# pengpeng-yu/FastPCC

Measured on AMD Instinct MI355X. Metric: encode+decode Mpoints/sec, lossy_coord_v2 baseline_r1 (stream of 16-frame batches, 2 in flight; one frame at a time = value_one_frame), higher is better.
Workload: dtype f32; 1 GPU; lossy_coord_v2/baseline_r1 inference, 997645-voxel 1024^3 body-surface frames (cfg#2), seeded random-init weights; one step = a batch of 16 such frames per GPU (15966320 voxels) through compress_many + decompress_many = ONE network traversal over the batch, 16 independent streams; 2 batch(es) in flight per GPU; parallelism=single GPU, 2 batches in flight per GPU on one stream (fastpcc_amd/serving.py), batch_clouds=16, frames_in_flight=2, named_stages=False, bytes=143901, coder_handover_retries=0

## Files before the change

fastpcc_amd/csrc/hip/conv.hip:

```cpp
#include "conv_common.h"
#include <atomic>
#include <cstdlib>

namespace fpcc {
namespace {

template <int NBT, int CH, int WM, int WN>
struct MfmaCfg {
    static constexpr int C_OUT = 32 * NBT;
    static constexpr int TM = 32 * WM;
    static constexpr int NBW = NBT / WN;
    static constexpr int THREADS = 64 * WM * WN;
    static constexpr int G8 = CH / 8;
    static constexpr int W_TOTAL = CH * C_OUT / 4;
    static constexpr int W_PIECES = (W_TOTAL + THREADS - 1) / THREADS;
    static_assert(NBT % WN == 0, "column blocks must divide over the waves");
};

template <typename C, int CH>
__device__ __forceinline__ void fetch_a(const ConvArgs &a, const int32_t *nbr_rows, int cc, int li, int lh,
                                        f32x4 (&ra)[C::G8]) {
    const bool in_x1 = cc * CH < a.c1;
    const float *xb = in_x1 ? a.x1 + cc * CH : a.x2 + (cc * CH - a.c1);
    const int64_t ld = in_x1 ? a.ld1 : a.ld2;
    const int32_t idx = nbr_rows[li];
// ... 1591 lines not shown
    }
    if (ch == 32) {
        if (c_out == 128) return launch_mfma<4, 32>(a, s);
        if (c_out == 64) return launch_mfma<2, 32>(a, s);
        return launch_mfma<1, 32>(a, s);
    }
    if (ch == 16) {
        if (c_out == 128) return launch_mfma<4, 16>(a, s);
        if (c_out == 64) return launch_mfma<2, 16>(a, s);
        return launch_mfma<1, 16>(a, s);
    }
    if (c1 == 1 && c2 == 0 && n_offsets == 1 && !nbr && groups == 1 && !out_map && c_out >= 8) {
        hipLaunchKernelGGL(k_conv_c1_pointwise, dim3(blocks_for(n_out * c_out, 256)), dim3(256), 0, s, a);
        return check_hip(hipGetLastError(), "k_conv_c1_pointwise");
    }
    if (c_out == 1) return launch_valu<1>(a, s);
    if (c_out <= 4) return launch_valu<4>(a, s);
    if (c_out <= 8) return launch_valu<8>(a, s);
    return launch_valu<16>(a, s);
}

namespace fpcc {
namespace {
__global__ void k_conv_row_keys(const int32_t *__restrict__ nbr, int n_off, int64_t nbr_ks, int64_t nbr_os, int64_t n,
                                int window_log2, int64_t *__restrict__ keys, uint32_t *__restrict__ masks) {
    const int64_t o = (int64_t)blockIdx.x * blockDim.x + threadIdx.x;
    if (o >= n) return;
    uint32_t m = 0;
    for (int k = 0; k < n_off; ++k) m |= (nbr[(int64_t)k * nbr_ks + o * nbr_os] >= 0 ? 1u : 0u) << k;
    if (masks) masks[o] = m;
    m ^= m >> 1; m ^= m >> 2; m ^= m >> 4; m ^= m >> 8; m ^= m >> 16;
    keys[o] = ((o >> window_log2) << 32) | (int64_t)m;
}

__global__ void k_conv_row_keys_masks(const uint32_t *__restrict__ masks, int64_t n, int window_log2, int64_t *__restrict__ keys) {
    const int64_t o = (int64_t)blockIdx.x * blockDim.x + threadIdx.x;
    if (o >= n) return;
    uint32_t m = masks[o];
    m ^= m >> 1; m ^= m >> 2; m ^= m >> 4; m ^= m >> 8; m ^= m >> 16;
    keys[o] = ((o >> window_log2) << 32) | (int64_t)m;
}

__global__ __launch_bounds__(256) void k_gather_table_rows(const int4 *__restrict__ rows, const int32_t *__restrict__ order, int64_t n,
                                                           int pieces, int4 *__restrict__ out) {
    const int64_t e = (int64_t)blockIdx.x * 256 + threadIdx.x;
    if (e >= n * pieces) return;
    const int64_t p = e / pieces;
    const int j = (int)(e - p * pieces);
    out[e] = rows[(int64_t)order[p] * pieces + j];
}

__global__ __launch_bounds__(256) void k_conv_tile_keys(const uint32_t *__restrict__ row_masks, int n_off,
                                                        const int32_t *__restrict__ row_order, int64_t n, int group,
                                                        int64_t n_groups, int64_t *__restrict__ keys) {
    const int64_t g = (int64_t)blockIdx.x * 4 + (threadIdx.x >> 6);
    const int lane = threadIdx.x & 63;
    if (g >= n_groups) return;
    const int64_t pos = g * group + lane;
    uint32_t m = 0;
    if (lane < group && pos < n) m = row_masks[row_order ? (int64_t)row_order[pos] : pos];
#pragma unroll
    for (int o = 32; o > 0; o >>= 1) m |= __shfl_xor(m, o);
    if (lane == 0) keys[g] = ((int64_t)(n_off - __popc(m)) << 32) | g;
}
// ... 41 lines not shown
    __syncthreads();
#pragma unroll
    for (int j = 0; j < kPer; ++j) {
        if (bin[j] == 255) continue;
        uint32_t pos = 0;
#pragma unroll
        for (int b = 0; b < kBins; ++b)
            if (bin[j] == b) { pos = s_base[b] + s_wave[wv][b] + before[b]; before[b] += 1; }
        perm[pos] = g0 + j;
    }
}

__global__ void k_conv_regroup_rows(const int32_t *__restrict__ row_order, const int32_t *__restrict__ group_perm, int64_t n,
                                    int group, int64_t n_groups, int32_t *__restrict__ out) {
    const int64_t p = (int64_t)blockIdx.x * blockDim.x + threadIdx.x;
    if (p >= n) return;
    const int64_t g = p / group;
    const int64_t src = g < n_groups ? (int64_t)group_perm[g] * group + (p - g * group) : p;
    out[p] = row_order ? row_order[src] : (int32_t)src;
}
}
}

extern "C" int fpcc_conv_tile_keys(const uint32_t *row_masks, int n_offsets, const int32_t *row_order, int64_t n, int group,
                                   int64_t *keys_out, void *stream) {
    if (n < 0 || n_offsets < 1 || n_offsets > 32 || group < 1 || group > 64) return fail_arg("conv_tile_keys: sizes out of range");
    const int64_t n_groups = n / group;
    if (n_groups == 0) return FPCC_OK;
    if (!row_masks || !keys_out) return fail_arg("conv_tile_keys: null pointer");
    hipLaunchKernelGGL(k_conv_tile_keys, dim3(blocks_for(n_groups, 4)), dim3(256), 0, as_stream(stream), row_masks, n_offsets,
                       row_order, n, group, n_groups, keys_out);
    return check_hip(hipGetLastError(), "k_conv_tile_keys");
}

extern "C" int fpcc_conv_group_order(const int64_t *group_keys, int64_t n_groups, int32_t *perm_out, void *stream) {
    if (n_groups < 0 || n_groups > 16384) return fail_arg("conv_group_order: at most 16384 groups");
    if (n_groups == 0) return FPCC_OK;
    if (!group_keys || !perm_out) return fail_arg("conv_group_order: null pointer");
    const int per = (int)((n_groups + 1023) / 1024);
    if (per <= 2) hipLaunchKernelGGL(k_group_counting_order<2>, dim3(1), dim3(1024), 0, as_stream(stream), group_keys, (int)n_groups, perm_out);
    else if (per <= 5) hipLaunchKernelGGL(k_group_counting_order<5>, dim3(1), dim3(1024), 0, as_stream(stream), group_keys, (int)n_groups, perm_out);
    else hipLaunchKernelGGL(k_group_counting_order<16>, dim3(1), dim3(1024), 0, as_stream(stream), group_keys, (int)n_groups, perm_out);
    return check_hip(hipGetLastError(), "k_group_counting_order");
}

extern "C" int fpcc_conv_regroup_rows(const int32_t *row_order, const int32_t *group_perm, int64_t n, int group,
                                      int32_t *row_order_out, void *stream) {
    if (n < 0 || group < 1) return fail_arg("conv_regroup_rows: sizes out of range");
    if (n == 0) return FPCC_OK;
    if (!row_order_out || (n / group > 0 && !group_perm)) return fail_arg("conv_regroup_rows: null pointer");
    hipLaunchKernelGGL(k_conv_regroup_rows, dim3(blocks_for(n, 256)), dim3(256), 0, as_stream(stream), row_order, group_perm, n,
                       group, n / group, row_order_out);
    return check_hip(hipGetLastError(), "k_conv_regroup_rows");
}

extern "C" int fpcc_conv_row_keys_masks(const uint32_t *masks, int64_t n, int window_log2, int64_t *keys_out, void *stream) {
    if (n < 0 || window_log2 < 5 || window_log2 > 31) return fail_arg("conv_row_keys_masks: bad sizes");
    if (n == 0) return FPCC_OK;
    if (!masks || !keys_out) return fail_arg("conv_row_keys_masks: null pointer");
    hipLaunchKernelGGL(k_conv_row_keys_masks, dim3(blocks_for(n, 256)), dim3(256), 0, as_stream(stream), masks, n, window_log2, keys_out);
    return check_hip(hipGetLastError(), "k_conv_row_keys_masks");
}

extern "C" int fpcc_gather_table_rows_i32(const int32_t *rows, int ld, const int32_t *order, int64_t n, int32_t *out, void *stream) {
    if (n < 0 || ld < 4 || ld % 4) return fail_arg("gather_table_rows: ld must be a positive multiple of 4");
    if (n == 0) return FPCC_OK;
    if (!rows || !order || !out || !aligned16(rows) || !aligned16(out)) return fail_arg("gather_table_rows: null or unaligned pointer");
    hipLaunchKernelGGL(k_gather_table_rows, dim3(blocks_for(n * (ld / 4), 256)), dim3(256), 0, as_stream(stream),
                       reinterpret_cast<const int4 *>(rows), order, n, ld / 4, reinterpret_cast<int4 *>(out));
    return check_hip(hipGetLastError(), "k_gather_table_rows");
}

extern "C" int fpcc_conv_row_keys(const int32_t *nbr, int n_offsets, int64_t nbr_ks, int64_t nbr_os, int64_t n,
                                  int window_log2, int64_t *keys_out, uint32_t *masks_out, void *stream) {
    if (n < 0 || n_offsets < 1 || n_offsets > 32 || window_log2 < 5 || window_log2 > 30)
        return fail_arg("conv_row_keys: sizes out of range");
    if (n == 0) return FPCC_OK;
    if (!nbr || !keys_out) return fail_arg("conv_row_keys: null pointer");
    hipLaunchKernelGGL(k_conv_row_keys, dim3(blocks_for(n, 256)), dim3(256), 0, as_stream(stream), nbr, n_offsets, nbr_ks,
                       nbr_os, n, window_log2, keys_out, masks_out);
    return check_hip(hipGetLastError(), "k_conv_row_keys");
}

namespace fpcc {
namespace {
constexpr int64_t kK2s2tSparseRows = 200 * 1024;
std::atomic<long long> g_k2s2t_sparse_launches{0};

__global__ __launch_bounds__(1024) void k_k2s2t_order(const int32_t *__restrict__ parent_of, const int32_t *__restrict__ child_row,
                                                      int64_t n, int64_t n_parents, int window_log2, int32_t *__restrict__ order,
                                                      int32_t *__restrict__ table) {
    __shared__ uint32_t s_cnt[16][8];
    __shared__ uint32_t s_base[2][8];
    const int t = threadIdx.x, lane = t & 63, wv = t >> 6;
    const int64_t w0 = (int64_t)blockIdx.x << window_log2;
    const int64_t w1 = min(n, w0 + ((int64_t)1 << window_log2));
    auto octant_of = [&](int64_t c, int32_t &par) {
        par = parent_of[c];
        if (par < 0 || par >= n_parents) { par = -1; return 0; }
        const int4 *line = reinterpret_cast<const int4 *>(child_row + (int64_t)par * 8);
        const int4 lo = line[0], hi = line[1];
        const int32_t e[8] = {lo.x, lo.y, lo.z, lo.w, hi.x, hi.y, hi.z, hi.w};
        int o = -1;
#pragma unroll
// ... 234 lines not shown
```

fastpcc_amd/engine.py:

```python
import functools
import math
import os
from enum import Enum
from typing import Dict, List, Optional, Sequence, Tuple, Union

import torch
import torch.nn as nn

from . import hipops as ops
from .autograd import conv_autocast


class RegionType(Enum):
    HYPER_CUBE = 0
    HYPER_CROSS = 1
    CUSTOM = 2


class MinkowskiAlgorithm(Enum):
    DEFAULT = 0
    MEMORY_EFFICIENT = 1
    SPEED_OPTIMIZED = 2


# ... 152 lines not shown
            raise KeyError(f'{key} is not in this coordinate manager') from None

    def get_coordinate_map_keys(self, tensor_stride) -> List[CoordinateMapKey]:
        s = _as_stride(tensor_stride)
        return [k for k in self._maps if k._stride == s]

    def insert_and_map(self, coordinates: torch.Tensor, tensor_stride=1, string_id: str = ''):
        stride = _as_stride(tensor_stride)
        level = stride[0].bit_length() - 1
        if coordinates.dtype != torch.int32 or coordinates.dim() != 2 or coordinates.shape[1] != 4:
            raise TypeError('coordinates must be int32 [n, 4] = (batch, x, y, z)')
        coordinates = coordinates.contiguous()
        self.device = coordinates.device
        if self._bits0 is None:
            nb = self._n_batch
            if nb is None:
                nb = int(coordinates[:, 0].max().item()) + 1 if coordinates.shape[0] else 1
            self._n_batch = nb
            self._bits0 = min(21, (63 - max(nb - 1, 0).bit_length()) // 3)
        bits = self._bits0 - level
        if bits < 1:
            raise ValueError('tensor stride exceeds the coordinate range')
        keys = ops.keys_from_coords(coordinates, level, bits)
        skeys, perm = ops.sort_keys(keys, 63)
        ukeys, first, count = ops.unique_keys(skeys)
        n = int(count.item())
        m = _Map(level, bits, n, ukeys[:n])
        rows = perm if n == coordinates.shape[0] else perm[first[:n].long()]
        key = self._register(m, string_id)
        return key, (rows, n)

    def _ensure_parent(self, m: _Map, rows: Optional[int] = None, edges: Optional[List[int]] = None) -> _Map:
        if m.parent is None:
            if m.bits <= 1:
                raise ValueError('cannot stride past the coordinate range')
            parent_of, pkeys, child_row, count = ops.coarsen(self._keys(m))
            cnt = int(count.item()) if rows is None else rows
            p = _Map(m.level + 1, m.bits - 1, cnt, pkeys[:cnt])
            p.edges = edges
            m.parent, m.parent_of, m.child_row = p, parent_of, child_row[:cnt]
            self._register(p, '')
        return m.parent

    def build_pyramid(self, key: CoordinateMapKey, levels: int) -> None:
        m = self._map(key)
        while m.parent is not None and levels > 0:
            m, levels = m.parent, levels - 1
# ... 94 lines not shown
        return dict(nbr=m.nbr27_pos, n_offsets=27, nbr_ks=1, nbr_os=32)

    def _mask27(self, m: _Map) -> Optional[torch.Tensor]:
        if m.mask27 is None:
            if m.generated or m.nbr27 is not None:
                return None
            if m.parent is None and m.n > self.ROOT_ROWS and m.bits > 1:
                self._ensure_parent(m)
            if m.parent is None:
                return None
            m.mask27 = ops.mask27_from_parent(m.keys, m.parent_of, self._nbr27(m.parent, True), m.child_row)
        return m.mask27

    ROW_ORDER_MIN_ROWS = int(os.environ.get('FPCC_ROW_ORDER_MIN_ROWS', '8192'))
    ROW_ORDER_WINDOW_LOG2 = int(os.environ.get('FPCC_ROW_WINDOW_LOG2', '19'))

    ROW_ORDER_MIN_ROWS_TRAINING = 512

    def _row_order(self, m: _Map, training: bool = False) -> Optional[torch.Tensor]:
        if m.row_order is False or (m.row_order is None and training and m.n > self.ROW_ORDER_MIN_ROWS_TRAINING):
            m.row_order = None
            if m.n > (self.ROW_ORDER_MIN_ROWS_TRAINING if training else self.ROW_ORDER_MIN_ROWS):
                nbr = self._nbr27(m, want_rows=not training)
                m.row_order = ops.conv_row_order(nbr, 27, m.n, 1, m.n, self.ROW_ORDER_WINDOW_LOG2,
                                                 masks=m.mask27 if m.nbr27_rows is not None else None)
        return m.row_order

    def _k2_order(self, src: _Map):
        m = src.parent.n
        if src.k2_order is False:
            src.k2_order = None
            if self.NBR_ROWS and m > self.ROW_ORDER_MIN_ROWS and os.environ.get('FPCC_K2_ROW_ORDER', '1') != '0':
                src.k2_order = ops.conv_row_order(src.child_row, 8, 1, 8, m, self.ROW_ORDER_WINDOW_LOG2)
                src.k2_pos = ops.gather_table_rows(src.child_row, src.k2_order)
        if src.k2_order is None:
            return None, src.child_row
        return src.k2_order, src.k2_pos

    K2T_WINDOW_LOG2 = ops.K2S2T_WINDOW_LOG2

    def _k2t_order(self, dst: _Map):
        if dst.k2t_order is False:
            dst.k2t_order = None
            po, cr = dst.parent_of, dst.child_row
            if dst.n > 0 and po is not None and cr is not None and dst.parent is not None and po.numel() == dst.n and \
                    po.dtype == torch.int32 and cr.dtype == torch.int32 and cr.dim() == 2 and tuple(cr.shape) == (dst.parent.n, 8) and \
                    po.is_contiguous() and cr.is_contiguous():
                dst.k2t_order, dst.k2t_table = ops.conv_k2s2t_order(po, cr, dst.n, self.K2T_WINDOW_LOG2)
        return dst.k2t_order, dst.k2t_table

    def get_coordinates(self, key: CoordinateMapKey) -> torch.Tensor:
        m = self._map(key)
        if m.coords is None:
            m.coords = ops.coords_from_keys(self._keys(m), m.level, m.bits)
        return m.coords

    def kernel_map(self, in_key: CoordinateMapKey, out_key: CoordinateMapKey, stride=1, kernel_size=1, **_):
# ... 625 lines not shown
```

fastpcc_amd/hipops.py:

```python
import collections
import ctypes as C
import functools
from typing import List, Optional, Sequence, Tuple

import torch

from . import _native

_vp, _i64, _i32, _f32 = C.c_void_p, C.c_int64, C.c_int, C.c_float

ACT_NONE, ACT_PRELU, ACT_RELU = 0, 1, 2

_SIGS = {
    'fpcc_morton3d_encode': (_i32, [_vp, _i64, _i64, _i32, _i32, _i32, _vp, _vp]),
    'fpcc_hilbert3d_encode': (_i32, [_vp, _i64, _i64, _i32, _i32, _i32, _i32, _vp, _vp]),
    'fpcc_keys_from_coords': (_i32, [_vp, _i64, _i32, _i32, _vp, _vp]),
    'fpcc_coords_from_keys': (_i32, [_vp, _i64, _i32, _i32, _vp, _vp, _vp]),
    'fpcc_sort_keys': (_i64, [_vp, _i64, _i32, _vp, _vp, _vp, _i64, _vp]),
    'fpcc_unique_keys': (_i64, [_vp, _i64, _vp, _vp, _vp, _vp, _i64, _vp]),
    'fpcc_coarsen': (_i64, [_vp, _i64, _vp, _vp, _vp, _vp, _vp, _i64, _vp]),
    'fpcc_octree_level': (_i64, [_vp, _i64, _i64, _i32, _vp, _vp, _vp, _vp, _i64, _vp, _vp, _i64, _vp]),
    'fpcc_level_histogram': (_i64, [_vp, _i64, _i32, _vp, _vp]),
    'fpcc_level_histogram_clouds': (_i64, [_vp, _i64, _i32, _i32, _i32, _vp, _vp]),
    'fpcc_refine': (_i64, [_vp, _i64, _vp, _vp, _vp, _vp, _vp, _vp, _i64, _vp]),
    'fpcc_nbr27_search': (_i32, [_vp, _i64, _i32, _vp, _vp]),
    'fpcc_nbr27_from_parent': (_i32, [_vp, _vp, _i64, _vp, _i64, _vp, _vp, _vp]),
    'fpcc_nbr27_from_parent_ex': (_i32, [_vp, _vp, _i64, _vp, _i64, _vp, _vp, _vp, _vp, _vp]),
    'fpcc_conv_row_keys_masks': (_i32, [_vp, _i64, _i32, _vp, _vp]),
    'fpcc_gather_table_rows_i32': (_i32, [_vp, _i32, _vp, _i64, _vp, _vp]),
    'fpcc_mask27_from_parent': (_i32, [_vp, _vp, _i64, _vp, _i64, _vp, _vp, _vp]),
    'fpcc_conv_ones_k3_f32': (_i32, [_vp, _i64, _vp, _vp, _i32, _i32, _vp, C.c_float, _vp, _i32, _vp]),
    'fpcc_conv_f32': (_i32, [_vp, _i32, _i32, _vp, _i32, _i32, _vp, _i32, _i64, _i64, _vp, _vp, _i32, _i32,
                             _vp, _i64, _i64, _vp, _i32, _i64, _i32, _vp, _f32, _vp, _vp, _i64, _vp]),
    'fpcc_conv_f32_pk': (_i32, [_vp, _i32, _i32, _vp, _i32, _i32, _vp, _i32, _i64, _i64, _vp, _vp, _vp, _i32, _i32,
                                _vp, _i64, _i64, _vp, _i32, _i64, _i32, _vp, _f32, _vp, _vp, _i64, _vp]),
    'fpcc_conv_set_tuning': (_i32, [_i32, _i32]),
    'fpcc_conv_fold64_launches': (_i64, []),
    'fpcc_conv_k2s2t_order': (_i32, [_vp, _vp, _i64, _i64, _i32, _vp, _vp, _vp]),
    'fpcc_conv_k2s2t_f32': (_i32, [_vp, _i32, _i32, _vp, _vp, _vp, _vp, _i32, _vp, _i32, _i64, _i32, _vp, _f32, _vp]),
    'fpcc_conv_k2s2t_use_sparse': (_i32, [_i32, _i32, _i64]),
    'fpcc_conv_k2s2t_sparse_launches': (_i64, []),
    'fpcc_conv_debug_stamps': (_i32, [_vp, _i64]),
    'fpcc_conv_i8_debug_stamps': (_i32, [_vp, _i64]),
    'fpcc_time_next_launch': (_i32, [_vp, _vp]),
    'fpcc_transpose_table_i32': (_i32, [_vp, _i32, _i64, _vp, _i32, _vp]),
    'fpcc_numerics_version': (_i32, []),
    'fpcc_conv_packed_floats': (_i64, [_i32, _i32, _i32, _i32, _i32]),
    'fpcc_conv_pack_weights_f32': (_i32, [_vp, _i64, _i32, _i32, _vp, _vp]),
    'fpcc_conv_f32_natural_matrix': (_i32, [_i32, _i32, _i32, _i32, _i32]),
    'fpcc_conv_packed_floats_nat': (_i64, [_i32, _i32, _i32, _i32, _i32]),
    'fpcc_conv_pack_weights_nat_f32': (_i32, [_vp, _i64, _i32, _i32, _vp, _vp]),
# ... 2 lines not shown
    'fpcc_nn_dist2': (_i32, [_vp, _i64, _i32, _vp, _i64, _vp, _vp, _vp]),
    'fpcc_knn3d': (_i32, [_vp, _i64, _vp, _i64, _i32, _vp, _vp, _vp]),
    'fpcc_sum_i64': (_i32, [_vp, _i64, _vp, _vp]),
    'fpcc_knn_voxels': (_i32, [_vp, _i64, _i32, _vp, _i64, _i32, _i32, _vp, _vp, _vp]),
    'fpcc_pca_normals': (_i32, [_vp, _i64, _i32, _vp, _i64, _i32, _vp, _vp]),
    'fpcc_nn_plane_dist2': (_i32, [_vp, _i64, _i32, _vp, _vp, _i64, _vp, _vp, _vp, _vp]),
    'fpcc_transfer_normals_ws_bytes': (_i64, [_i64, _i64]),
    'fpcc_transfer_normals': (_i32, [_vp, _i64, _vp, _vp, _vp, _i64, _vp, _i32, _vp, _vp, _i64, _vp]),
    'fpcc_sum_max_f64': (_i32, [_vp, _i64, _vp, _vp, _i64, _vp]),
    'fpcc_recolor_ws_bytes': (_i64, [_i64]),
    'fpcc_recolor': (_i32, [_vp, _i64, _vp, _i64, _vp, _i32, _vp, _vp, _i64, _vp]),
    'fpcc_keys_member': (_i32, [_vp, _i64, _vp, _i64, _vp, _vp]),
    'fpcc_transpose_weights_f32': (_i32, [_vp, _i32, _i32, _i32, _i32, _vp, _vp]),
    'fpcc_conv_wgrad_ws_bytes': (_i64, [_i32, _i32, _i32, _i32, _i64]),
    'fpcc_conv_wgrad_f32': (_i32, [_vp, _i32, _i32, _vp, _i32, _i32, _vp, _i32, _i64, _i64, _vp, _i64, _i64, _i32, _i64, _vp, _vp,
                                   _i32, _vp, _i64, _vp]),
    'fpcc_conv_wgrad_matrix': (_i32, [_i32, _i32]),
    'fpcc_epilogue_bwd_ws_bytes': (_i64, [_i64, _i32]),
    'fpcc_epilogue_bwd_f32': (_i32, [_vp, _i32, _vp, _i32, _i64, _i32, _i32, _vp, _vp, _i32, _vp, _vp, _vp, _i64, _vp]),
    'fpcc_noisy_normal_ws_bytes': (_i64, [_i64]),
    'fpcc_noisy_normal_bits_f32': (_i32, [_vp, _vp, _i64, _f32, _f32, _f32, _vp, _vp, _vp, _vp, _i64, _vp]),
    'fpcc_deep_factorized_ws_bytes': (_i64, [_i64, _i32]),
    'fpcc_deep_factorized_bits_f32': (_i32, [_vp, _i64, _i32, _i32, _vp, _vp, _vp, _f32, _vp, _i32, _vp, _vp, _i64, _vp]),
    'fpcc_conv_tile_keys': (_i32, [_vp, _i32, _vp, _i64, _i32, _vp, _vp]),
    'fpcc_conv_regroup_rows': (_i32, [_vp, _vp, _i64, _i32, _vp, _vp]),
    'fpcc_conv_group_order': (_i32, [_vp, _i64, _vp, _vp]),
    'fpcc_conv_row_keys': (_i32, [_vp, _i32, _i64, _i64, _i64, _i32, _vp, _vp, _vp]),
    'fpcc_conv_f32_ws_bytes': (_i64, [_i32, _i32, _i32, _i32, _i32, _i64]),
    'fpcc_conv_f32_order': (_i32, [_i32, _i32, _i32]),
    'fpcc_conv_f32_order_ex': (_i32, [_i32, _i32, _i32, _i32, _i32, _i64]),
    'fpcc_conv_f32_plan': (_i32, [_i32, _i32, _i32, _i32, _i32, _vp]),
    'fpcc_gather_sum_f32': (_i32, [_vp, _i32, _vp, _i32, _i64, _i64, _i64, _vp, _i32, _vp, _f32, _vp, _vp]),
    'fpcc_gather_sum_generated_f32': (_i32, [_vp, _i32, _vp, _i64, _vp, _i32, _vp, _f32, _vp, _vp]),
    'fpcc_logit_to_prob16': (_i32, [_vp, _i64, _vp, _vp]),
    'fpcc_quantize_symbols': (_i32, [_vp, _i64, _f32, _vp, _vp]),
    'fpcc_child_mask': (_i32, [_vp, _i64, _vp, _vp]),
    'fpcc_topk_keep': (_i64, [_vp, _i64, _i64, _vp, _vp, _i64, _vp]),
    'fpcc_topk_keep_cells': (_i64, [_vp, _i64, _vp, _i64, _i64, _vp, _vp, _i64, _vp]),
    'fpcc_topk_keep_batch': (_i64, [_vp, _i64, _vp, _i32, _vp, _i64, _vp, _vp, _vp, _i64, _vp]),
    'fpcc_gather_rows_f32': (_i32, [_vp, _i32, _i32, _vp, _i64, _vp, _i32, _vp]),
    'fpcc_compact_coords': (_i64, [_vp, _i64, _vp, _i32, _i32, _vp, _vp, _vp, _vp, _i64, _vp]),
    'fpcc_int_init': (_i32, []),
    'fpcc_hash_insert_coords': (_i32, [_vp, _vp, _i64, _vp, _i64, _vp]),
    'fpcc_hash_lookup_coords': (_i32, [_vp, _vp, _i64, _vp, _i64, _vp, _vp, _vp, _vp]),
    'fpcc_hash_insert_coords_bxyz': (_i32, [_vp, _vp, _i64, _vp, _i64, _vp]),
    'fpcc_hash_lookup_coords_bxyz': (_i32, [_vp, _vp, _i64, _vp, _i64, _vp, _vp, _vp, _vp]),
    'fpcc_hash_insert_keys': (_i32, [_vp, _vp, _i64, _vp, _i64, _vp]),
    'fpcc_hash_lookup_keys': (_i32, [_vp, _vp, _i64, _vp, _i64, _vp, _vp]),
    'fpcc_conv_i8': (_i32, [_vp, _i32, _i32, _vp, _i32, _i64, _i64, _i32, _vp, _i32, _vp, _vp, _vp, _vp, _vp, _i32, _i32,
                            _vp, _i32, _i32, _i32, _i64, _vp, _vp, _i64, _vp]),
# ... 931 lines not shown
                                        None if dy is None else dy.data_ptr(), c, out.data_ptr(), ws.data_ptr(), need, _stream()))
    return out, dy


def noisy_normal_bits(y: torch.Tensor, index: torch.Tensor, log_scale_offset: float, log_scale_factor: float,
                      half_width: float = 0.5):
    n = y.numel()
    if index.numel() != n:
        raise ValueError('one index per value')
    index = index.to(torch.float32)
    py, pi = _dev(y, torch.float32, 'y', n == 0), _dev(index, torch.float32, 'index', n == 0)
    dy = torch.empty(n, dtype=torch.float32, device=y.device)
    di = torch.empty(n, dtype=torch.float32, device=y.device)
    out = torch.empty(1, dtype=torch.float32, device=y.device)
    L = lib()
    need = _ok(L.fpcc_noisy_normal_ws_bytes(n))
    ws = torch.empty(max(need // 4, 1), dtype=torch.float32, device=y.device)
    _ok(L.fpcc_noisy_normal_bits_f32(py, pi, n, float(log_scale_offset), float(log_scale_factor), float(half_width),
                                     dy.data_ptr(), di.data_ptr(), out.data_ptr(), ws.data_ptr(), need, _stream()))
    return out[0], dy, di


def conv_row_order(nbr: Optional[torch.Tensor], n_offsets: int, nbr_ks: int, nbr_os: int, n: int, window_log2: int = 13,
                   heaviest_first: bool = True, masks: Optional[torch.Tensor] = None) -> torch.Tensor:
    L = lib()
    dev = masks.device if masks is not None else nbr.device
    keys = torch.empty(n, dtype=torch.int64, device=dev)
    group = 64 if n >= 32 * 1024 else 32
    n_groups = n // group
    heaviest_first = heaviest_first and 2 <= n_groups <= LPT_MAX_GROUPS
    if masks is not None:
        _ok(L.fpcc_conv_row_keys_masks(_dev(masks, torch.int32, 'masks'), n, window_log2, keys.data_ptr(), _stream()))
    else:
        masks = torch.empty(n, dtype=torch.int32, device=dev) if heaviest_first else None
        _ok(L.fpcc_conv_row_keys(_dev(nbr, torch.int32, 'nbr'), n_offsets, nbr_ks, nbr_os, n, window_log2, keys.data_ptr(),
                                 None if masks is None else masks.data_ptr(), _stream()))
    order = sort_keys(keys, 32 + max(1, (n >> window_log2).bit_length()))[1]
    if not heaviest_first:
        return order
    gkeys = torch.empty(n_groups, dtype=torch.int64, device=dev)
    _ok(L.fpcc_conv_tile_keys(masks.data_ptr(), n_offsets, order.data_ptr(), n, group, gkeys.data_ptr(), _stream()))
    gperm = torch.empty(n_groups, dtype=torch.int32, device=dev)
    _ok(L.fpcc_conv_group_order(gkeys.data_ptr(), n_groups, gperm.data_ptr(), _stream()))
    out = torch.empty_like(order)
    _ok(L.fpcc_conv_regroup_rows(order.data_ptr(), gperm.data_ptr(), n, group, out.data_ptr(), _stream()))
    return out


LPT_MAX_GROUPS = 1 << 14

def table_conv_chunk(c_in: int, c_out: int, k: int) -> int:
    mfma = conv_order(c_in, 0, c_out, 1, 1, 0) != 0
    if not mfma:
        return 32
    return k if k <= 27 else 16


class ConvPlan(C.Structure):
    _fields_ = [('order', _i32), ('matrix', _i32), ('packed', _i32), ('chunk', _i32), ('packed_floats', _i64), ('ws_bytes', _i64)]


ConvPlanValue = collections.namedtuple('ConvPlanValue', [f for f, _ in ConvPlan._fields_])


@functools.lru_cache(maxsize=8192)
def conv_plan(c1: int, c2: int, c_out: int, n_offsets: int = 1, groups: int = 1) -> ConvPlanValue:
    plan = ConvPlan()
    _ok(lib().fpcc_conv_f32_plan(c1, c2, c_out, n_offsets, groups, C.byref(plan)))
    return ConvPlanValue(*(getattr(plan, f) for f in ConvPlanValue._fields))


def conv_order(c1: int, c2: int, c_out: int, n_offsets: int = 1, groups: int = 1, n_out: int = 0) -> int:
# ... 476 lines not shown
```

include/fpcc_hip.h:

```cpp
#ifndef FPCC_HIP_H_
#define FPCC_HIP_H_
#include <stdint.h>
#ifdef __cplusplus
extern "C" {
#endif

typedef enum {
    FPCC_OK = 0,
    FPCC_E_ARG = -1,
    FPCC_E_HIP = -2,
    FPCC_E_WORKSPACE = -3
} fpcc_status;

const char *fpcc_last_error(void);
int fpcc_device_count(void);
int fpcc_clock_probe(int64_t *out2, int spin_us, void *stream);


int fpcc_morton3d_encode(const int32_t *coords, int64_t n, int64_t row_stride, int col_bit0, int col_bit1, int col_bit2,
                         int64_t *keys_out, void *stream);

int fpcc_hilbert3d_encode(const int32_t *coords, int64_t n, int64_t row_stride, int col_x, int col_y, int col_z, int bits,
                          int64_t *keys_out, void *stream);

// ... 70 lines not shown
typedef struct {
    const float *w;
    const float *w_packed;
    const float *bias;
    const float *slope;
    int c_out;
    int act;
    float clip;
} fpcc_mlp_layer;
typedef struct {
    const float *x; int cx; int ldx;
    const float *y; int cy; int ldy;
    int cat_layer;
    int n_layers;
    fpcc_mlp_layer layers[FPCC_MLP_CHAIN_MAX_LAYERS];
    float *out; int ldo;
    int64_t n;
} fpcc_mlp_chain;
int fpcc_mlp_chain_f32(const fpcc_mlp_chain *chain, void *stream);
int fpcc_mlp_chain_set_form(int form);
int fpcc_pointwise_head_f32(const float *x, int c0, int ldx, const float *w1, const float *b1, int c1, int act1,
                            const float *slope1, int order1, const float *w2, const float *b2, int act2, const float *slope2,
                            float clip, float *out, int64_t n, void *stream);
int fpcc_conv_row_keys(const int32_t *nbr, int n_offsets, int64_t nbr_ks, int64_t nbr_os, int64_t n, int window_log2,
                       int64_t *keys_out, uint32_t *masks_out, void *stream);
int fpcc_conv_row_keys_masks(const uint32_t *masks, int64_t n, int window_log2, int64_t *keys_out, void *stream);
int fpcc_gather_table_rows_i32(const int32_t *rows, int ld, const int32_t *order, int64_t n, int32_t *out, void *stream);
int fpcc_conv_tile_keys(const uint32_t *row_masks, int n_offsets, const int32_t *row_order, int64_t n, int group,
                        int64_t *keys_out, void *stream);
int fpcc_conv_group_order(const int64_t *group_keys, int64_t n_groups, int32_t *perm_out, void *stream);
int fpcc_conv_regroup_rows(const int32_t *row_order, const int32_t *group_perm, int64_t n, int group, int32_t *row_order_out,
                           void *stream);
typedef struct fpcc_conv_plan {
    int32_t order;
    int32_t matrix;
    int32_t packed;
    int32_t chunk;
    int64_t packed_floats;
    int64_t ws_bytes;
} fpcc_conv_plan;
int fpcc_conv_f32_plan(int c1, int c2, int c_out, int n_offsets, int groups, fpcc_conv_plan *plan);
int64_t fpcc_conv_f32_ws_bytes(int c1, int c2, int c_out, int n_offsets, int groups, int64_t n_out);
int fpcc_conv_f32_order(int c1, int c2, int c_out);
int fpcc_conv_f32_order_ex(int c1, int c2, int c_out, int n_offsets, int groups, int64_t n_out);

int64_t fpcc_conv_wgrad_ws_bytes(int c_in, int c_out, int n_offsets, int groups, int64_t n);
int fpcc_conv_wgrad_f32(const float *x, int c_in, int ldx, const float *dy, int c_out, int ldy,
                        const int32_t *nbr, int n_offsets, int64_t nbr_ks, int64_t nbr_os,
                        const int32_t *out_map, int64_t om_os, int64_t om_gs, int groups, int64_t n,
                        const int32_t *row_order, float *dw, int accumulate, void *ws, int64_t ws_bytes, void *stream);
int fpcc_conv_wgrad_matrix(int c_in, int c_out);
int fpcc_transpose_weights_f32(const float *w, int n_offsets, int c_in, int c_out, int flip, float *wt, void *stream);

int64_t fpcc_epilogue_bwd_ws_bytes(int64_t n, int c);
int fpcc_epilogue_bwd_f32(const float *y, int ldy, const float *dy, int lddy, int64_t n, int c, int act, const float *slope,
// ... 165 lines not shown
```

profiles/hbm_bandwidth_by_size.py:

```python
#!/usr/bin/env python3
import collections
import csv
import os
import sys

KERNELS = ('k_nbr27_from_parent<false>', 'k_nbr27_from_parent<true>', 'k_nbr27_from_parent<2>', 'k_nbr27_from_parent<1>', 'k_nbr27_from_parent<0>',
           'k_gather_sum_generated', 'k_gather_sum', 'k_gather_table_rows', 'k_coarsen_scatter', 'k_refine_scatter',
           'k_conv_row_keys', 'k_conv_row_keys_masks', 'k_pointwise_head', 'k_conv_ones_k3', 'k_unique_scatter', 'k_logit_to_prob16', 'k_child_mask')


def counters(d):
    by = collections.defaultdict(list)
    with open(os.path.join(d, 'p_counter_collection.csv')) as f:
        for r in csv.DictReader(f):
            by[r['Kernel_Name']].append((int(r['Dispatch_Id']), float(r['Counter_Value'])))
    return {k: [v for _, v in sorted(rows)] for k, rows in by.items()}


def durations(d):
    by = collections.defaultdict(list)
    with open(os.path.join(d, 'p_kernel_trace.csv')) as f:
        for r in csv.DictReader(f):
            by[r['Kernel_Name']].append((int(r['Dispatch_Id']), (int(r['End_Timestamp']) - int(r['Start_Timestamp'])) / 1e3))
    return {k: [v for _, v in sorted(rows)] for k, rows in by.items()}


def main(fetch_dir, write_dir):
    fetch, write, dur = counters(fetch_dir), counters(write_dir), durations(fetch_dir)
    print('| kernel | launches | all launches, TB/s | largest sixth, TB/s | largest launch | % of 8 TB/s (largest) |')
    print('|---|---:|---:|---:|---|---:|')
    for key in KERNELS:
# ... 17 lines not shown
```

Before: 92.44 Mpoints/s.

## Fuse conv row-order pipeline into one native call with narrow 32-bit radix sort

```diff
diff --git a/fastpcc_amd/csrc/hip/conv.hip b/fastpcc_amd/csrc/hip/conv.hip
--- a/fastpcc_amd/csrc/hip/conv.hip
+++ b/fastpcc_amd/csrc/hip/conv.hip
@@ -1,6 +1,7 @@
 #include "conv_common.h"
 #include <atomic>
 #include <cstdlib>
+#include <rocprim/device/device_radix_sort.hpp>
 
 namespace fpcc {
 namespace {
@@ -1638,24 +1639,40 @@
 
 namespace fpcc {
 namespace {
-__global__ void k_conv_row_keys(const int32_t *__restrict__ nbr, int n_off, int64_t nbr_ks, int64_t nbr_os, int64_t n,
-                                int window_log2, int64_t *__restrict__ keys, uint32_t *__restrict__ masks) {
+__device__ __forceinline__ uint32_t row_mask(const uint32_t *__restrict__ masks_in, const int32_t *__restrict__ nbr, int n_off,
+                                             int64_t nbr_ks, int64_t nbr_os, int64_t o, uint32_t *__restrict__ masks_out) {
+    if (masks_in) return masks_in[o];
+    uint32_t m = 0;
+    for (int k = 0; k < n_off; ++k) m |= (nbr[(int64_t)k * nbr_ks + o * nbr_os] >= 0 ? 1u : 0u) << k;
+    if (masks_out) masks_out[o] = m;
+    return m;
+}
+
+__device__ __forceinline__ uint32_t gray_rank(uint32_t m) {
+    m ^= m >> 1; m ^= m >> 2; m ^= m >> 4; m ^= m >> 8; m ^= m >> 16;
+    return m;
+}
+
+__global__ void k_conv_row_keys64(const uint32_t *__restrict__ masks_in, const int32_t *__restrict__ nbr, int n_off, int64_t nbr_ks,
+                                  int64_t nbr_os, int64_t n, int window_log2, int64_t *__restrict__ keys,
+                                  uint32_t *__restrict__ masks_out) {
     const int64_t o = (int64_t)blockIdx.x * blockDim.x + threadIdx.x;
     if (o >= n) return;
-    uint32_t m = 0;
-    for (int k = 0; k < n_off; ++k) m |= (nbr[(int64_t)k * nbr_ks + o * nbr_os] >= 0 ? 1u : 0u) << k;
-    if (masks) masks[o] = m;
-    m ^= m >> 1; m ^= m >> 2; m ^= m >> 4; m ^= m >> 8; m ^= m >> 16;
-    keys[o] = ((o >> window_log2) << 32) | (int64_t)m;
-}
-
-__global__ void k_conv_row_keys_masks(const uint32_t *__restrict__ masks, int64_t n, int window_log2, int64_t *__restrict__ keys) {
+    const uint32_t m = row_mask(masks_in, nbr, n_off, nbr_ks, nbr_os, o, masks_out);
+    keys[o] = ((o >> window_log2) << 32) | (int64_t)gray_rank(m);
+}
+
+__global__ void k_conv_row_keys32(const uint32_t *__restrict__ masks_in, const int32_t *__restrict__ nbr, int n_off, int64_t nbr_ks,
+                                  int64_t nbr_os, int64_t n, int window_log2, uint32_t *__restrict__ keys, int32_t *__restrict__ rows,
+                                  uint32_t *__restrict__ masks_out) {
     const int64_t o = (int64_t)blockIdx.x * blockDim.x + threadIdx.x;
     if (o >= n) return;
-    uint32_t m = masks[o];
-    m ^= m >> 1; m ^= m >> 2; m ^= m >> 4; m ^= m >> 8; m ^= m >> 16;
-    keys[o] = ((o >> window_log2) << 32) | (int64_t)m;
-}
+    const uint32_t m = row_mask(masks_in, nbr, n_off, nbr_ks, nbr_os, o, masks_out);
+    keys[o] = ((uint32_t)(o >> window_log2) << n_off) | gray_rank(m);
+    rows[o] = (int32_t)o;
+}
+
+constexpr int64_t kLptMaxGroups = 16384;
 
 __global__ __launch_bounds__(256) void k_gather_table_rows(const int4 *__restrict__ rows, const int32_t *__restrict__ order, int64_t n,
                                                            int pieces, int4 *__restrict__ out) {
@@ -1743,44 +1760,19 @@
 }
 }
 
-extern "C" int fpcc_conv_tile_keys(const uint32_t *row_masks, int n_offsets, const int32_t *row_order, int64_t n, int group,
-                                   int64_t *keys_out, void *stream) {
-    if (n < 0 || n_offsets < 1 || n_offsets > 32 || group < 1 || group > 64) return fail_arg("conv_tile_keys: sizes out of range");
-    const int64_t n_groups = n / group;
-    if (n_groups == 0) return FPCC_OK;
-    if (!row_masks || !keys_out) return fail_arg("conv_tile_keys: null pointer");
-    hipLaunchKernelGGL(k_conv_tile_keys, dim3(blocks_for(n_groups, 4)), dim3(256), 0, as_stream(stream), row_masks, n_offsets,
-                       row_order, n, group, n_groups, keys_out);
-    return check_hip(hipGetLastError(), "k_conv_tile_keys");
+static int launch_group_order(const int64_t *group_keys, int64_t n_groups, int32_t *perm_out, hipStream_t s) {
+    const int per = (int)((n_groups + 1023) / 1024);
+    if (per <= 2) hipLaunchKernelGGL(k_group_counting_order<2>, dim3(1), dim3(1024), 0, s, group_keys, (int)n_groups, perm_out);
+    else if (per <= 5) hipLaunchKernelGGL(k_group_counting_order<5>, dim3(1), dim3(1024), 0, s, group_keys, (int)n_groups, perm_out);
+    else hipLaunchKernelGGL(k_group_counting_order<16>, dim3(1), dim3(1024), 0, s, group_keys, (int)n_groups, perm_out);
+    return check_hip(hipGetLastError(), "k_group_counting_order");
 }
 
 extern "C" int fpcc_conv_group_order(const int64_t *group_keys, int64_t n_groups, int32_t *perm_out, void *stream) {
-    if (n_groups < 0 || n_groups > 16384) return fail_arg("conv_group_order: at most 16384 groups");
+    if (n_groups < 0 || n_groups > kLptMaxGroups) return fail_arg("conv_group_order: at most 16384 groups");
     if (n_groups == 0) return FPCC_OK;
     if (!group_keys || !perm_out) return fail_arg("conv_group_order: null pointer");
-    const int per = (int)((n_groups + 1023) / 1024);
-    if (per <= 2) hipLaunchKernelGGL(k_group_counting_order<2>, dim3(1), dim3(1024), 0, as_stream(stream), group_keys, (int)n_groups, perm_out);
-    else if (per <= 5) hipLaunchKernelGGL(k_group_counting_order<5>, dim3(1), dim3(1024), 0, as_stream(stream), group_keys, (int)n_groups, perm_out);
-    else hipLaunchKernelGGL(k_group_counting_order<16>, dim3(1), dim3(1024), 0, as_stream(stream), group_keys, (int)n_groups, perm_out);
-    return check_hip(hipGetLastError(), "k_group_counting_order");
-}
-
-extern "C" int fpcc_conv_regroup_rows(const int32_t *row_order, const int32_t *group_perm, int64_t n, int group,
-                                      int32_t *row_order_out, void *stream) {
-    if (n < 0 || group < 1) return fail_arg("conv_regroup_rows: sizes out of range");
-    if (n == 0) return FPCC_OK;
-    if (!row_order_out || (n / group > 0 && !group_perm)) return fail_arg("conv_regroup_rows: null pointer");
-    hipLaunchKernelGGL(k_conv_regroup_rows, dim3(blocks_for(n, 256)), dim3(256), 0, as_stream(stream), row_order, group_perm, n,
-                       group, n / group, row_order_out);
-    return check_hip(hipGetLastError(), "k_conv_regroup_rows");
-}
-
-extern "C" int fpcc_conv_row_keys_masks(const uint32_t *masks, int64_t n, int window_log2, int64_t *keys_out, void *stream) {
-    if (n < 0 || window_log2 < 5 || window_log2 > 31) return fail_arg("conv_row_keys_masks: bad sizes");
-    if (n == 0) return FPCC_OK;
-    if (!masks || !keys_out) return fail_arg("conv_row_keys_masks: null pointer");
-    hipLaunchKernelGGL(k_conv_row_keys_masks, dim3(blocks_for(n, 256)), dim3(256), 0, as_stream(stream), masks, n, window_log2, keys_out);
-    return check_hip(hipGetLastError(), "k_conv_row_keys_masks");
+    return launch_group_order(group_keys, n_groups, perm_out, as_stream(stream));
 }
 
 extern "C" int fpcc_gather_table_rows_i32(const int32_t *rows, int ld, const int32_t *order, int64_t n, int32_t *out, void *stream) {
@@ -1792,15 +1784,90 @@
     return check_hip(hipGetLastError(), "k_gather_table_rows");
 }
 
-extern "C" int fpcc_conv_row_keys(const int32_t *nbr, int n_offsets, int64_t nbr_ks, int64_t nbr_os, int64_t n,
-                                  int window_log2, int64_t *keys_out, uint32_t *masks_out, void *stream) {
-    if (n < 0 || n_offsets < 1 || n_offsets > 32 || window_log2 < 5 || window_log2 > 30)
-        return fail_arg("conv_row_keys: sizes out of range");
+using RowSortFewBits = rocprim::radix_sort_config<rocprim::default_config, rocprim::default_config, rocprim::default_config, 16 * 1024>;
+using RowSortManyBits = rocprim::radix_sort_config<rocprim::default_config, rocprim::default_config, rocprim::default_config, 256 * 1024>;
+static hipError_t sort_pairs32(void *tmp, size_t &bytes, const uint32_t *k_in, uint32_t *k_out, const int32_t *r_in, int32_t *r_out,
+                               size_t n, unsigned end_bit, hipStream_t s) {
+    if (end_bit <= 16) return rocprim::radix_sort_pairs<RowSortFewBits>(tmp, bytes, k_in, k_out, r_in, r_out, n, 0u, end_bit, s);
+    return rocprim::radix_sort_pairs<RowSortManyBits>(tmp, bytes, k_in, k_out, r_in, r_out, n, 0u, end_bit, s);
+}
+
+extern "C" int64_t fpcc_conv_row_order(const uint32_t *masks, const int32_t *nbr, int n_offsets, int64_t nbr_ks, int64_t nbr_os,
+                                       int64_t n, int window_log2, int group, int heaviest_first, int32_t *order_out,
+                                       const int32_t *rows, int ld, int32_t *rows_out, void *ws, int64_t ws_bytes, void *stream) {
+    if (n < 0 || n > INT32_MAX || n_offsets < 1 || n_offsets > 32 || window_log2 < 5 || window_log2 > 30 || group < 0 || group > 64)
+        return fail_arg("conv_row_order: sizes out of range");
+    if (group == 0) group = n >= 32 * 1024 ? 64 : 32;
+    const int64_t n_groups = n / group;
+    const bool heaviest = heaviest_first && n_groups >= 2 && n_groups <= kLptMaxGroups;
+    int window_bits = 1;
+    while ((n >> window_log2) >> window_bits) ++window_bits;
+    const bool narrow = window_bits + n_offsets <= 32;
+    const int end_bit = (narrow ? n_offsets : 32) + ((n >> window_log2) == 0 ? 0 : window_bits);
+
+    const int64_t nn = n > 0 ? n : 1;
+    const int64_t words = align_up(4 * nn, 256);
+    const int64_t gkeys_bytes = align_up(8 * (n_groups > 0 ? n_groups : 1), 256);
+    const int64_t gperm_bytes = align_up(4 * (n_groups > 0 ? n_groups : 1), 256);
+    int64_t sort_bytes = 0;
+    if (!narrow) {
+        sort_bytes = fpcc_sort_keys(nullptr, n, end_bit, nullptr, nullptr, nullptr, 0, nullptr);
+        if (sort_bytes < 0) return sort_bytes;
+    } else {
+        size_t bytes = 0;
+        FPCC_HIP(sort_pairs32(nullptr, bytes, nullptr, nullptr, nullptr, nullptr, (size_t)nn, (unsigned)end_bit, nullptr));
+        sort_bytes = align_up((int64_t)bytes, 256);
+    }
+    const int64_t key_bytes = narrow ? 3 * words : 2 * align_up(8 * nn, 256);
+    const int64_t need = 2 * words + gkeys_bytes + gperm_bytes + key_bytes + sort_bytes;
+    if (!ws) return need;
+    if (ws_bytes < need) { set_error("conv_row_order: workspace %lld < %lld", (long long)ws_bytes, (long long)need); return FPCC_E_WORKSPACE; }
     if (n == 0) return FPCC_OK;
-    if (!nbr || !keys_out) return fail_arg("conv_row_keys: null pointer");
-    hipLaunchKernelGGL(k_conv_row_keys, dim3(blocks_for(n, 256)), dim3(256), 0, as_stream(stream), nbr, n_offsets, nbr_ks,
-                       nbr_os, n, window_log2, keys_out, masks_out);
-    return check_hip(hipGetLastError(), "k_conv_row_keys");
+    if (!order_out || (!masks && !nbr)) return fail_arg("conv_row_order: null pointer");
+    if (rows && (ld < 4 || ld % 4 || !rows_out || !aligned16(rows) || !aligned16(rows_out)))
+        return fail_arg("conv_row_order: the table needs ld a positive multiple of 4 and 16-byte aligned pointers");
+
+    char *w = static_cast<char *>(ws);
+    uint32_t *masks_tmp = reinterpret_cast<uint32_t *>(w);      w += words;
+    int32_t *order_tmp = reinterpret_cast<int32_t *>(w);        w += words;
+    int64_t *gkeys = reinterpret_cast<int64_t *>(w);            w += gkeys_bytes;
+    int32_t *gperm = reinterpret_cast<int32_t *>(w);            w += gperm_bytes;
+    char *keys = w;                                             w += key_bytes;
+    void *sort_ws = w;
+    hipStream_t s = as_stream(stream);
+    uint32_t *masks_out = (!masks && heaviest) ? masks_tmp : nullptr;
+    int32_t *sorted = heaviest ? order_tmp : order_out;
+
+    if (narrow) {
+        uint32_t *k_in = reinterpret_cast<uint32_t *>(keys), *k_out = reinterpret_cast<uint32_t *>(keys + words);
+        int32_t *r_in = reinterpret_cast<int32_t *>(keys + 2 * words);
+        hipLaunchKernelGGL(k_conv_row_keys32, dim3(blocks_for(n, 256)), dim3(256), 0, s, masks, nbr, n_offsets, nbr_ks, nbr_os, n,
+                           window_log2, k_in, r_in, masks_out);
+        FPCC_LAUNCHED(k_conv_row_keys32);
+        size_t bytes = (size_t)sort_bytes;
+        FPCC_HIP(sort_pairs32(sort_ws, bytes, k_in, k_out, r_in, sorted, (size_t)n, (unsigned)end_bit, s));
+    } else {
+        int64_t *k_in = reinterpret_cast<int64_t *>(keys), *k_out = reinterpret_cast<int64_t *>(keys + align_up(8 * nn, 256));
+        hipLaunchKernelGGL(k_conv_row_keys64, dim3(blocks_for(n, 256)), dim3(256), 0, s, masks, nbr, n_offsets, nbr_ks, nbr_os, n,
+                           window_log2, k_in, masks_out);
+        FPCC_LAUNCHED(k_conv_row_keys64);
+        if (int64_t rc = fpcc_sort_keys(k_in, n, end_bit, k_out, sorted, sort_ws, sort_bytes, stream)) return rc;
+    }
+    if (heaviest) {
+        hipLaunchKernelGGL(k_conv_tile_keys, dim3(blocks_for(n_groups, 4)), dim3(256), 0, s, masks ? masks : masks_tmp, n_offsets,
+                           (const int32_t *)sorted, n, group, n_groups, gkeys);
+        FPCC_LAUNCHED(k_conv_tile_keys);
+        if (int rc = launch_group_order(gkeys, n_groups, gperm, s)) return rc;
+        hipLaunchKernelGGL(k_conv_regroup_rows, dim3(blocks_for(n, 256)), dim3(256), 0, s, (const int32_t *)sorted,
+                           (const int32_t *)gperm, n, group, n_groups, order_out);
+        FPCC_LAUNCHED(k_conv_regroup_rows);
+    }
+    if (rows) {
+        hipLaunchKernelGGL(k_gather_table_rows, dim3(blocks_for(n * (ld / 4), 256)), dim3(256), 0, s,
+                           reinterpret_cast<const int4 *>(rows), (const int32_t *)order_out, n, ld / 4, reinterpret_cast<int4 *>(rows_out));
+        FPCC_LAUNCHED(k_gather_table_rows);
+    }
+    return FPCC_OK;
 }
 
 namespace fpcc {
diff --git a/fastpcc_amd/engine.py b/fastpcc_amd/engine.py
--- a/fastpcc_amd/engine.py
+++ b/fastpcc_amd/engine.py
@@ -198,7 +198,7 @@
         if bits < 1:
             raise ValueError('tensor stride exceeds the coordinate range')
         keys = ops.keys_from_coords(coordinates, level, bits)
-        skeys, perm = ops.sort_keys(keys, 63)
+        skeys, perm = ops.sort_keys(keys, max(1, max(self._n_batch - 1, 0).bit_length() + 3 * bits))
         ukeys, first, count = ops.unique_keys(skeys)
         n = int(count.item())
         m = _Map(level, bits, n, ukeys[:n])
@@ -339,8 +339,12 @@
             m.row_order = None
             if m.n > (self.ROW_ORDER_MIN_ROWS_TRAINING if training else self.ROW_ORDER_MIN_ROWS):
                 nbr = self._nbr27(m, want_rows=not training)
-                m.row_order = ops.conv_row_order(nbr, 27, m.n, 1, m.n, self.ROW_ORDER_WINDOW_LOG2,
-                                                 masks=m.mask27 if m.nbr27_rows is not None else None)
+                if m.nbr27_rows is not None and m.nbr27_pos is None:
+                    m.row_order, m.nbr27_pos = ops.conv_row_order(nbr, 27, m.n, 1, m.n, self.ROW_ORDER_WINDOW_LOG2,
+                                                                  masks=m.mask27, rows=m.nbr27_rows)
+                    m.nbr27_rows = None
+                else:
+                    m.row_order = ops.conv_row_order(nbr, 27, m.n, 1, m.n, self.ROW_ORDER_WINDOW_LOG2)
         return m.row_order
 
     def _k2_order(self, src: _Map):
@@ -348,8 +352,8 @@
         if src.k2_order is False:
             src.k2_order = None
             if self.NBR_ROWS and m > self.ROW_ORDER_MIN_ROWS and os.environ.get('FPCC_K2_ROW_ORDER', '1') != '0':
-                src.k2_order = ops.conv_row_order(src.child_row, 8, 1, 8, m, self.ROW_ORDER_WINDOW_LOG2)
-                src.k2_pos = ops.gather_table_rows(src.child_row, src.k2_order)
+                src.k2_order, src.k2_pos = ops.conv_row_order(src.child_row, 8, 1, 8, m, self.ROW_ORDER_WINDOW_LOG2,
+                                                              rows=src.child_row)
         if src.k2_order is None:
             return None, src.child_row
         return src.k2_order, src.k2_pos
diff --git a/fastpcc_amd/hipops.py b/fastpcc_amd/hipops.py
--- a/fastpcc_amd/hipops.py
+++ b/fastpcc_amd/hipops.py
@@ -26,7 +26,6 @@
     'fpcc_nbr27_search': (_i32, [_vp, _i64, _i32, _vp, _vp]),
     'fpcc_nbr27_from_parent': (_i32, [_vp, _vp, _i64, _vp, _i64, _vp, _vp, _vp]),
     'fpcc_nbr27_from_parent_ex': (_i32, [_vp, _vp, _i64, _vp, _i64, _vp, _vp, _vp, _vp, _vp]),
-    'fpcc_conv_row_keys_masks': (_i32, [_vp, _i64, _i32, _vp, _vp]),
     'fpcc_gather_table_rows_i32': (_i32, [_vp, _i32, _vp, _i64, _vp, _vp]),
     'fpcc_mask27_from_parent': (_i32, [_vp, _vp, _i64, _vp, _i64, _vp, _vp, _vp]),
     'fpcc_conv_ones_k3_f32': (_i32, [_vp, _i64, _vp, _vp, _i32, _i32, _vp, C.c_float, _vp, _i32, _vp]),
@@ -75,10 +74,8 @@
     'fpcc_noisy_normal_bits_f32': (_i32, [_vp, _vp, _i64, _f32, _f32, _f32, _vp, _vp, _vp, _vp, _i64, _vp]),
     'fpcc_deep_factorized_ws_bytes': (_i64, [_i64, _i32]),
     'fpcc_deep_factorized_bits_f32': (_i32, [_vp, _i64, _i32, _i32, _vp, _vp, _vp, _f32, _vp, _i32, _vp, _vp, _i64, _vp]),
-    'fpcc_conv_tile_keys': (_i32, [_vp, _i32, _vp, _i64, _i32, _vp, _vp]),
-    'fpcc_conv_regroup_rows': (_i32, [_vp, _vp, _i64, _i32, _vp, _vp]),
     'fpcc_conv_group_order': (_i32, [_vp, _i64, _vp, _vp]),
-    'fpcc_conv_row_keys': (_i32, [_vp, _i32, _i64, _i64, _i64, _i32, _vp, _vp, _vp]),
+    'fpcc_conv_row_order': (_i64, [_vp, _vp, _i32, _i64, _i64, _i64, _i32, _i32, _i32, _vp, _vp, _i32, _vp, _vp, _i64, _vp]),
     'fpcc_conv_f32_ws_bytes': (_i64, [_i32, _i32, _i32, _i32, _i32, _i64]),
     'fpcc_conv_f32_order': (_i32, [_i32, _i32, _i32]),
     'fpcc_conv_f32_order_ex': (_i32, [_i32, _i32, _i32, _i32, _i32, _i64]),
@@ -1056,32 +1053,23 @@
 
 
 def conv_row_order(nbr: Optional[torch.Tensor], n_offsets: int, nbr_ks: int, nbr_os: int, n: int, window_log2: int = 13,
-                   heaviest_first: bool = True, masks: Optional[torch.Tensor] = None) -> torch.Tensor:
+                   heaviest_first: bool = True, masks: Optional[torch.Tensor] = None, rows: Optional[torch.Tensor] = None):
     L = lib()
     dev = masks.device if masks is not None else nbr.device
-    keys = torch.empty(n, dtype=torch.int64, device=dev)
-    group = 64 if n >= 32 * 1024 else 32
-    n_groups = n // group
-    heaviest_first = heaviest_first and 2 <= n_groups <= LPT_MAX_GROUPS
-    if masks is not None:
-        _ok(L.fpcc_conv_row_keys_masks(_dev(masks, torch.int32, 'masks'), n, window_log2, keys.data_ptr(), _stream()))
-    else:
-        masks = torch.empty(n, dtype=torch.int32, device=dev) if heaviest_first else None
-        _ok(L.fpcc_conv_row_keys(_dev(nbr, torch.int32, 'nbr'), n_offsets, nbr_ks, nbr_os, n, window_log2, keys.data_ptr(),
-                                 None if masks is None else masks.data_ptr(), _stream()))
-    order = sort_keys(keys, 32 + max(1, (n >> window_log2).bit_length()))[1]
-    if not heaviest_first:
-        return order
-    gkeys = torch.empty(n_groups, dtype=torch.int64, device=dev)
-    _ok(L.fpcc_conv_tile_keys(masks.data_ptr(), n_offsets, order.data_ptr(), n, group, gkeys.data_ptr(), _stream()))
-    gperm = torch.empty(n_groups, dtype=torch.int32, device=dev)
-    _ok(L.fpcc_conv_group_order(gkeys.data_ptr(), n_groups, gperm.data_ptr(), _stream()))
-    out = torch.empty_like(order)
-    _ok(L.fpcc_conv_regroup_rows(order.data_ptr(), gperm.data_ptr(), n, group, out.data_ptr(), _stream()))
-    return out
-
-
-LPT_MAX_GROUPS = 1 << 14
+    order = torch.empty(n, dtype=torch.int32, device=dev)
+    pm = None if masks is None else _dev(masks, torch.int32, 'masks', n == 0)
+    pn = None if masks is not None else _dev(nbr, torch.int32, 'nbr', n == 0)
+    pr, ld, out = None, 0, None
+    if rows is not None:
+        if rows.dim() != 2 or rows.shape[0] != n:
+            raise ValueError('rows must be [n, ld]')
+        pr, ld, out = _dev(rows, torch.int32, 'rows', n == 0), rows.shape[1], torch.empty_like(rows)
+    args = (pm, pn, n_offsets, nbr_ks, nbr_os, n, window_log2, 0, int(bool(heaviest_first)), order.data_ptr(), pr, ld,
+            None if out is None else out.data_ptr())
+    ws, need = _ws(lambda: L.fpcc_conv_row_order(*args, None, 0, None), dev)
+    _ok(L.fpcc_conv_row_order(*args, ws.data_ptr(), need, _stream()))
+    return order if rows is None else (order, out)
+
 
 def table_conv_chunk(c_in: int, c_out: int, k: int) -> int:
     mfma = conv_order(c_in, 0, c_out, 1, 1, 0) != 0
diff --git a/include/fpcc_hip.h b/include/fpcc_hip.h
--- a/include/fpcc_hip.h
+++ b/include/fpcc_hip.h
@@ -116,15 +116,11 @@
 int fpcc_pointwise_head_f32(const float *x, int c0, int ldx, const float *w1, const float *b1, int c1, int act1,
                             const float *slope1, int order1, const float *w2, const float *b2, int act2, const float *slope2,
                             float clip, float *out, int64_t n, void *stream);
-int fpcc_conv_row_keys(const int32_t *nbr, int n_offsets, int64_t nbr_ks, int64_t nbr_os, int64_t n, int window_log2,
-                       int64_t *keys_out, uint32_t *masks_out, void *stream);
-int fpcc_conv_row_keys_masks(const uint32_t *masks, int64_t n, int window_log2, int64_t *keys_out, void *stream);
+int64_t fpcc_conv_row_order(const uint32_t *masks, const int32_t *nbr, int n_offsets, int64_t nbr_ks, int64_t nbr_os, int64_t n,
+                            int window_log2, int group, int heaviest_first, int32_t *order_out, const int32_t *rows, int ld,
+                            int32_t *rows_out, void *ws, int64_t ws_bytes, void *stream);
 int fpcc_gather_table_rows_i32(const int32_t *rows, int ld, const int32_t *order, int64_t n, int32_t *out, void *stream);
-int fpcc_conv_tile_keys(const uint32_t *row_masks, int n_offsets, const int32_t *row_order, int64_t n, int group,
-                        int64_t *keys_out, void *stream);
 int fpcc_conv_group_order(const int64_t *group_keys, int64_t n_groups, int32_t *perm_out, void *stream);
-int fpcc_conv_regroup_rows(const int32_t *row_order, const int32_t *group_perm, int64_t n, int group, int32_t *row_order_out,
-                           void *stream);
 typedef struct fpcc_conv_plan {
     int32_t order;
     int32_t matrix;
diff --git a/profiles/hbm_bandwidth_by_size.py b/profiles/hbm_bandwidth_by_size.py
--- a/profiles/hbm_bandwidth_by_size.py
+++ b/profiles/hbm_bandwidth_by_size.py
@@ -6,7 +6,7 @@
 
 KERNELS = ('k_nbr27_from_parent<false>', 'k_nbr27_from_parent<true>', 'k_nbr27_from_parent<2>', 'k_nbr27_from_parent<1>', 'k_nbr27_from_parent<0>',
            'k_gather_sum_generated', 'k_gather_sum', 'k_gather_table_rows', 'k_coarsen_scatter', 'k_refine_scatter',
-           'k_conv_row_keys', 'k_conv_row_keys_masks', 'k_pointwise_head', 'k_conv_ones_k3', 'k_unique_scatter', 'k_logit_to_prob16', 'k_child_mask')
+           'k_conv_row_keys32', 'k_conv_row_keys64', 'k_pointwise_head', 'k_conv_ones_k3', 'k_unique_scatter', 'k_logit_to_prob16', 'k_child_mask')
 
 
 def counters(d):
```

After: 92.34 Mpoints/s, median of 2. No clear change (-0.1%).
